# omnirevolve/omnirevolve-image-processor

Hardware: NVIDIA B200
Metric: megapixels/sec (resize+color+edge) (higher is better)
Workload: dtype u8

## Files before the change

### omnirevolve-image-processor_b200/csrc/capi.cu

```cuda
#include <stdlib.h>
#include "omni_internal.cuh"
#include "fast_kernels.cuh"
#include "fast_device.cuh"

#include <math.h>
#include <stdarg.h>
#include <stdio.h>
#include <string.h>

static thread_local char g_err[512] = "";

void omni_set_error(const char *fmt, ...)
{
    va_list ap;
    va_start(ap, fmt);
    vsnprintf(g_err, sizeof(g_err), fmt, ap);
    va_end(ap);
}

extern "C" const char *omni_last_error_string(void) { return g_err; }
extern "C" int omni_version(void) { return OMNI_ABI_VERSION; }

extern "C" int omni_device_count(void)
{
    int n = 0;
    if (cudaGetDeviceCount(&n) != cudaSuccess) { cudaGetLastError(); return 0; }
    return n;
}

extern "C" int omni_ctx_create(int device, omni_ctx **out)
{
    OMNI_REQUIRE(out != nullptr, "omni_ctx_create: out is NULL");
    int n = 0;
    cudaError_t e = cudaGetDeviceCount(&n);
    if (e != cudaSuccess || n == 0) {
        omni_set_error("no CUDA device available (%s); libomni_b200 has no CPU fallback",
                       e != cudaSuccess ? cudaGetErrorString(e) : "device count 0");
        cudaGetLastError();
        return OMNI_ERR_CUDA;
    }
    OMNI_REQUIRE(device >= 0 && device < n, "omni_ctx_create: device %d out of range [0,%d)", device, n);
    OMNI_CUDA(cudaSetDevice(device));
    omni_ctx *c = new omni_ctx();
    c->device = device;
    {
        const char *ev = getenv("OMNI_B200_EDGE_DENSE");
        c->edge_sparse = (ev && ev[0] == '1') ? 0 : 1;
        ev = getenv("OMNI_B200_ASSIGN_LABCELL");
        c->assign_rgbcell = (ev && ev[0] == '1') ? 0 : 1;
        ev = getenv("OMNI_B200_DENSE_PIPELINE");
        c->pipeline = (ev && ev[0] == '1') ? 0 : 1;
    }
    OMNI_CUDA(cudaMalloc(&c->d_flags, 64 * sizeof(int)));
    OMNI_CUDA(cudaMemset(c->d_flags, 0, 64 * sizeof(int)));
    OMNI_CUDA(cudaMalloc(&c->d_counts, 4 * OMNI_MAX_K * sizeof(unsigned long long)));
    OMNI_CUDA(cudaHostAlloc(&c->h_flags, 64 * sizeof(int), cudaHostAllocDefault));
    OMNI_CUDA(cudaHostAlloc(&c->h_counts, 4 * OMNI_MAX_K * sizeof(unsigned long long), cudaHostAllocDefault));
    OMNI_CUDA(cudaStreamCreateWithFlags(&c->stream, cudaStreamNonBlocking));
    OMNI_CUDA(cudaDeviceGetAttribute(&c->sm_count, cudaDevAttrMultiProcessorCount, device));
    *out = c;
    return OMNI_OK;
}

extern "C" int omni_ctx_destroy(omni_ctx *c)
{
    if (!c) return OMNI_OK;
    cudaSetDevice(c->device);
    for (int i = 0; i < OMNI_WS_SLOTS; i++) if (c->ws[i]) cudaFree(c->ws[i]);
    for (auto &kv : c->resize_tabs) if (kv.second.d_blob) cudaFree(kv.second.d_blob);
    if (c->d_flags) cudaFree(c->d_flags);
    if (c->d_rgb_boxes) cudaFree(c->d_rgb_boxes);
    if (c->d_rgb_boxes3) cudaFree(c->d_rgb_boxes3);
    if (c->d_counts) cudaFree(c->d_counts);
    if (c->h_flags) cudaFreeHost(c->h_flags);
    if (c->h_counts) cudaFreeHost(c->h_counts);
    if (c->stream) cudaStreamDestroy(c->stream);
    for (auto &r : c->prof) { cudaEventDestroy(r.a); cudaEventDestroy(r.b); }
    for (auto e : c->ev_pool) cudaEventDestroy(e);
    fast_ctx_release(c);
    if (c->pk_ready) {
        cudaStreamDestroy(c->pk_in); cudaStreamDestroy(c->pk_out);
        for (auto e : c->pk_ev) cudaEventDestroy(e);
    }
    if (c->pk_counts) cudaFreeHost(c->pk_counts);
    if (c->bd_ready) { for (auto e : c->bd_ev) cudaEventDestroy(e); cudaStreamDestroy(c->bd_tail); }
    if (c->band_helper) omni_ctx_destroy(c->band_helper);
    delete c;
    return OMNI_OK;
}

extern "C" int omni_set_fast_path(omni_ctx *ctx, int enable)
{
    OMNI_REQUIRE(ctx != nullptr, "omni_set_fast_path: ctx is NULL");
    ctx->fast = enable ? 1 : 0;
    if (enable) {
        ctx->edge_sparse = ctx->assign_rgbcell = (enable == 2) ? 0 : 1;
        ctx->pipeline = (enable == 1) ? 1 : 0;
    }
    return OMNI_OK;
}

extern "C" int omni_set_assume_binary_masks(omni_ctx *ctx, int enable)
{
    OMNI_REQUIRE(ctx != nullptr, "omni_set_assume_binary_masks: ctx is NULL");
    ctx->assume_binary = enable ? 1 : 0;
    return OMNI_OK;
}

extern "C" int omni_set_table_cache(omni_ctx *ctx, int enable)
{
    OMNI_REQUIRE(ctx != nullptr, "omni_set_table_cache: ctx is NULL");
    ctx->table_cache = enable ? 1 : 0;
    if (!enable) ctx->cells_valid = ctx->cells3_valid = 0;
    return OMNI_OK;
}

extern "C" int omni_set_host_bands(omni_ctx *ctx, int mode)
{
    OMNI_REQUIRE(ctx != nullptr, "ctx is NULL");
    OMNI_REQUIRE(mode >= 0 && mode <= 2, "omni_set_host_bands: mode must be 0, 1 or 2");
    ctx->host_bands = mode;
    return OMNI_OK;
}

extern "C" int omni_last_band_resends(omni_ctx *ctx) { return ctx ? ctx->last_band_resends : -1; }

extern "C" int omni_host_alloc(size_t bytes, void **out)
{
    OMNI_REQUIRE(out != nullptr, "omni_host_alloc: out is NULL");
    OMNI_CUDA(cudaHostAlloc(out, bytes ? bytes : 1, cudaHostAllocDefault));
    return OMNI_OK;
}

extern "C" int omni_host_free(void *p)
{
    if (p) OMNI_CUDA(cudaFreeHost(p));
    return OMNI_OK;
}

extern "C" int omni_last_hysteresis_passes(omni_ctx *ctx)
{
    if (!ctx) return 0;
    if (ctx->last_hyst_passes < 0) {
        cudaStream_t st = ctx->last_hyst_stream;
        if (cudaSetDevice(ctx->device) != cudaSuccess ||
            cudaMemcpyAsync(ctx->h_flags + 9, ctx->d_flags, sizeof(int), cudaMemcpyDeviceToHost, st) != cudaSuccess ||
            cudaStreamSynchronize(st) != cudaSuccess) {
            cudaGetLastError();
            return 0;
        }
        ctx->last_hyst_passes = ctx->h_flags[9];
    }
    return ctx->last_hyst_passes;
}

KScope::KScope(omni_ctx *ctx, const char *name, cudaStream_t s) : c(ctx), st(s)
// ... 903 lines not shown
```

### omnirevolve-image-processor_b200/csrc/fast_kernels.cu

```cuda
#include "fast_kernels.cuh"
#include "omni_tables.inc"
#include "fast_device.cuh"

#include <algorithm>
#include <type_traits>
#include <cooperative_groups.h>
#include <math.h>
#include <stdlib.h>
#include <string.h>
namespace cg = cooperative_groups;

#define FK_TRY(expr) do { int rc__ = (expr); if (rc__ != OMNI_OK) return rc__; } while (0)

__device__ u16 f_lab_tab[256 + 2048];
static bool f_tab_ready[64] = {false};

cudaError_t fast_tables()
{
    int dev = 0;
    cudaError_t e = cudaGetDevice(&dev);
    if (e != cudaSuccess) return e;
    if (dev < 64 && f_tab_ready[dev]) return cudaSuccess;
    e = cudaMemcpyToSymbol(f_lab_tab, OMNI_LAB_GAMMA, sizeof(OMNI_LAB_GAMMA), 0);
    if (e != cudaSuccess) return e;
// ... 798 lines not shown
                if (++run == R.maxt) emit();
            } else {
                if (run) emit();
                if (active && R.zero_fill) {
                    const int ty1 = min(y1, ty0 + ET_R);
                    for (int y = ty0; y < ty1; y++) {
                        const size_t o = (size_t)k * plane + (size_t)y * ws + c;
                        R.cbits[o] = 0u; R.sbits[o] = 0u;
                        if (R.edges) store_word_bytes(R.edges + (size_t)k * R.estride + (size_t)y * R.epitch, 32 * c, w, 0u, R.aligned16);
                    }
                }
            }
        }
        if (run) emit();
#pragma unroll
        for (int nt = 1; nt <= ET_MAXT; nt++) {
            int mine = 0;
            for (int i = 0; i < n_items; i++) mine += ((lens >> (3 * i)) & 7u) == (u32)nt;
            int x = mine;
#pragma unroll
            for (int d = 1; d < 32; d <<= 1) {
                int y = __shfl_up_sync(0xffffffffu, x, d);
                if (lane >= d) x += y;
            }
            const int total = __shfl_sync(0xffffffffu, x, 31);
            if (total == 0) continue;
            int base = 0;
            if (lane == 31) base = atomicAdd(R.run_counts + nt - 1, total);
            base = __shfl_sync(0xffffffffu, base, 31);
            int pos = base + x - mine;
            for (int i = 0; i < n_items; i++)
                if (((lens >> (3 * i)) & 7u) == (u32)nt) R.run_items[R.off.v[nt - 1] + pos++] = s_item[wid][i][lane];
        }
    }
}

static cudaError_t launch_morph(bool with02, int morph03, const u32 *in_bits, u32 *out_bits, const BitGeom &g, int K, u8 *masks,
                                size_t mstride, size_t mpitch, cudaStream_t st, int y_lo = 0, int y_hi = -1, const MorphRuns *runs = nullptr)
{
    if (y_hi < 0) y_hi = g.h;
    if (y_hi <= y_lo) return cudaSuccess;
    auto warps_at = [&](int tr) { return (long long)((g.ww + 127) / 128) * 4 * ((y_hi - y_lo + tr - 1) / tr) * K; };
    int tr = MORPH_TR;
    if (warps_at(MORPH_TR_BIG) >= MORPH_BIG_MIN_WARPS && (y_lo % MORPH_TR_BIG) == 0) tr = MORPH_TR_BIG;
    else if (warps_at(MORPH_TR_MID) >= MORPH_MID_MIN_WARPS && (y_lo % MORPH_TR_MID) == 0) tr = MORPH_TR_MID;
    dim3 b(128), grid((g.ww + 127) / 128, (y_hi - y_lo + tr - 1) / tr, K);
    int al = plane_align(masks, mstride, mpitch);
    MorphRuns R{};
    if (runs) R = *runs;
#define LM2(CODE, TAP, RUNS, TR) fk_morph<CODE, TAP, RUNS, TR><<<grid, b, 0, st>>>(in_bits, out_bits, g.ws, g.plane, g.h, g.w, masks, mstride, mpitch, al, y_lo, y_hi, R)
#define LM3(CODE, TAP, RUNS)                                                          \
    do {                                                                               \
        if (tr == MORPH_TR_BIG) LM2(CODE, TAP, RUNS, MORPH_TR_BIG);                    \
        else if (tr == MORPH_TR_MID) LM2(CODE, TAP, RUNS, MORPH_TR_MID);               \
        else LM2(CODE, TAP, RUNS, MORPH_TR);                                           \
    } while (0)
#define LM(CODE, TAP)                                                                  \
    do {                                                                               \
        if (runs) LM3(CODE, TAP, true); else LM3(CODE, TAP, false);                    \
    } while (0)
    if (with02) {
        switch (morph03) {
        case 0: LM(CODE_R_OC, 4); break;
        case 1: LM(CODE_F_O, 4); break;
        case 2: LM(CODE_F_C, 4); break;
        default: LM(CODE_F_OC, 4); break;
        }
    } else {
        switch (morph03) {
        case 1: LM(CODE_C_O, -1); break;
        case 2: LM(CODE_C_C, -1); break;
        case 3: LM(CODE_C_OC, -1); break;
        default: return cudaErrorInvalidValue;
        }
    }
#undef LM
#undef LM3
#undef LM2
    return cudaGetLastError();
}

#define HB_TR 32
#define HB_TW 32
#define HY_WORD_ROUNDS 4
#define HY_THREADS 1024

__device__ __forceinline__ void hy_patch_bytes(u8 *row, u32 promoted)
{
    if (row == nullptr) return;
    while (promoted) {
        int e = __ffs(promoted) - 1;
        promoted &= promoted - 1u;
        row[e] = 255;
    }
}

__device__ __forceinline__ int hy_worklist(u32 *__restrict__ ebits, const u32 *__restrict__ cbits, int ws, size_t plane, int h, int w, int n_weak,
                                   const u32 *__restrict__ worklist, u8 *__restrict__ edges, size_t estride, size_t epitch)
{
    const int wwl = (w + 31) >> 5;
    int rounds = 0;
    for (;;) {
        int changed = 0;
        for (int i = threadIdx.x; i < n_weak; i += HY_THREADS) {
            const u32 o = worklist[i];
            const int k = (int)(o / plane), rem = (int)(o - (size_t)k * plane);
            const int y = rem / ws, c = rem - y * ws;
            u32 *E = ebits + (size_t)k * plane + (size_t)y * ws;
            const u32 cv = __ldg(cbits + o);
            u32 m3[3], l3[3], r3[3];
#pragma unroll
            for (int dy = -1; dy <= 1; dy++) {
                const bool in = y + dy >= 0 && y + dy < h;
                const u32 *Er = E + (ptrdiff_t)dy * ws;
                m3[dy + 1] = in ? __ldcg(Er + c) : 0u;
                l3[dy + 1] = (in && c > 0) ? __ldcg(Er + c - 1) : 0u;
                r3[dy + 1] = (in && c + 1 < wwl) ? __ldcg(Er + c + 1) : 0u;
            }
            const u32 ev = m3[1];
            if ((cv & ~ev) == 0u) continue;
            u32 d = 0u;
#pragma unroll
            for (int q = 0; q < 3; q++) d |= m3[q] | (m3[q] << 1) | (m3[q] >> 1) | (l3[q] >> 31) | (r3[q] << 31);
            u32 nv = ev | (cv & d);
            for (;;) {
                u32 t = nv | (cv & ((nv << 1) | (nv >> 1)));
                if (t == nv) break;
                nv = t;
            }
            if (nv != ev) {
                E[c] = nv;
                changed = 1;
                hy_patch_bytes(edges ? edges + (size_t)k * estride + (size_t)y * epitch + 32 * c : nullptr, nv & ~ev);
            }
        }
        rounds++;
        __threadfence_block();
        if (!__syncthreads_or(changed)) break;
    }
    return rounds;
}

__global__ void __launch_bounds__(HY_THREADS) fk_hysteresis_wl(u32 *__restrict__ ebits, const u32 *__restrict__ cbits, int ws, size_t plane, int h,
                                                               int w, const int *flags, const u32 *__restrict__ worklist)
{
    const int n_weak = flags[4];
    if (n_weak > HY_WL_CAP) return;
    hy_worklist(ebits, cbits, ws, plane, h, w, n_weak, worklist, nullptr, 0, 0);
}

__global__ void __launch_bounds__(HY_THREADS) fk_hysteresis(u32 *__restrict__ ebits, const u32 *__restrict__ cbits, int ws, size_t plane, int h,
                                                     int w, int K, int *flags ,
                                                     const u32 *__restrict__ worklist,
                                                     u8 *__restrict__ edges, size_t estride, size_t epitch)
{
    cg::grid_group grid = cg::this_grid();
    const int n_weak = flags[4];
    if (n_weak <= HY_WL_CAP) {
        if (blockIdx.x != 0) return;
        const int rounds = hy_worklist(ebits, cbits, ws, plane, h, w, n_weak, worklist, edges, estride, epitch);
        if (threadIdx.x == 0) flags[0] = rounds;
        return;
    }
    __shared__ u32 s_e[(HB_TR + 2) * (HB_TW + 2)];
    __shared__ u32 s_c[HB_TR * HB_TW];
    const int ww = (w + 31) >> 5;
    const int tid = threadIdx.x;
    constexpr int SW = HB_TW + 2;
    int round = 0;
    for (;;) {
        volatile int *chg = flags + 1 + (round % 3);
        if (round < HY_WORD_ROUNDS) {
            const long long rows = (long long)K * h;
            const int lane = tid & 31;
            const long long warp0 = ((long long)blockIdx.x * blockDim.x + tid) >> 5, nwarps = ((long long)gridDim.x * blockDim.x) >> 5;
            for (long long R = warp0; R < rows; R += nwarps) {
                const int k = (int)(R / h), y = (int)(R - (long long)k * h);
                u32 *E = ebits + (size_t)k * plane + (size_t)y * ws;
                const u32 *C = cbits + (size_t)k * plane + (size_t)y * ws;
                for (int c = lane; c < ww; c += 32) {
                    const u32 cv = __ldg(C + c), ev = __ldcg(E + c);
                    if ((cv & ~ev) == 0u) continue;
                    u32 d = 0u;
#pragma unroll
                    for (int dy = -1; dy <= 1; dy++) {
                        if (y + dy < 0 || y + dy >= h) continue;
                        const u32 *Er = E + (ptrdiff_t)dy * ws;
                        u32 m = __ldcg(Er + c), l = c > 0 ? __ldcg(Er + c - 1) : 0u, r = c + 1 < ww ? __ldcg(Er + c + 1) : 0u;
                        d |= m | (m << 1) | (m >> 1) | (l >> 31) | (r << 31);
                    }
                    u32 nv = ev | (cv & d);
                    for (;;) {
                        u32 t = nv | (cv & ((nv << 1) | (nv >> 1)));
                        if (t == nv) break;
                        nv = t;
                    }
                    if (nv != ev) {
                        E[c] = nv;
                        *chg = 1;
                        hy_patch_bytes(edges ? edges + (size_t)k * estride + (size_t)y * epitch + 32 * c : nullptr, nv & ~ev);
                    }
                }
            }
        } else {
            const int tx_n = (ww + HB_TW - 1) / HB_TW, ty_n = (h + HB_TR - 1) / HB_TR;
            const int tiles = tx_n * ty_n * K;
            for (int t = blockIdx.x; t < tiles; t += gridDim.x) {
                const int k = t / (tx_n * ty_n), r = t - k * (tx_n * ty_n);
                const int ty = r / tx_n, tx = r - ty * tx_n;
                const int y0 = ty * HB_TR, c0 = tx * HB_TW;
                u32 *E = ebits + (size_t)k * plane;
                const u32 *C = cbits + (size_t)k * plane;
                int pending = 0;
                for (int i = tid; i < HB_TR * HB_TW; i += HY_THREADS) {
                    int ly = i / HB_TW, lc = i - ly * HB_TW;
                    int gy = y0 + ly, gc = c0 + lc;
                    u32 cv = 0, ev = 0;
                    if (gy < h && gc < ww) { cv = __ldg(C + (size_t)gy * ws + gc); ev = __ldcg(E + (size_t)gy * ws + gc); }
                    s_c[i] = cv;
                    s_e[(ly + 1) * SW + lc + 1] = ev;
                    pending |= (cv & ~ev) != 0;
                }
                if (!__syncthreads_or(pending)) continue;
                for (int i = tid; i < 2 * SW + 2 * HB_TR; i += HY_THREADS) {
                    int ly, lc;
                    if (i < SW) { ly = 0; lc = i; }
                    else if (i < 2 * SW) { ly = HB_TR + 1; lc = i - SW; }
                    else { int j = i - 2 * SW; ly = 1 + (j >> 1); lc = (j & 1) ? HB_TW + 1 : 0; }
                    int gy = y0 - 1 + ly, gc = c0 - 1 + lc;
                    s_e[ly * SW + lc] = (gy >= 0 && gy < h && gc >= 0 && gc < ww) ? __ldcg(E + (size_t)gy * ws + gc) : 0u;
                }
                __syncthreads();
                int any = 0;
                for (;;) {
                    int changed = 0;
                    for (int i = tid; i < HB_TR * HB_TW; i += HY_THREADS) {
                        int ly = i / HB_TW, lc = i - ly * HB_TW;
                        u32 cv = s_c[i];
                        int o = (ly + 1) * SW + lc + 1;
                        u32 ev = s_e[o];
                        if (cv & ~ev) {
                            u32 d = 0;
#pragma unroll
                            for (int dy = -1; dy <= 1; dy++) {
                                u32 l = s_e[o + dy * SW - 1], m = s_e[o + dy * SW], rr = s_e[o + dy * SW + 1];
                                d |= m | (m << 1) | (m >> 1) | (l >> 31) | (rr << 31);
                            }
                            u32 nv = ev | (cv & d);
                            if (nv != ev) { s_e[o] = nv; changed = 1; }
                        }
                    }
                    if (!__syncthreads_or(changed)) break;
                    any = 1;
                }
                if (any) {
                    for (int i = tid; i < HB_TR * HB_TW; i += HY_THREADS) {
                        int ly = i / HB_TW, lc = i - ly * HB_TW;
                        int gy = y0 + ly, gc = c0 + lc;
                        if (gy < h && gc < ww) {
                            u32 nv = s_e[(ly + 1) * SW + lc + 1], old = __ldcg(E + (size_t)gy * ws + gc);
                            if (nv & ~old) {
                                E[(size_t)gy * ws + gc] = nv | old;
                                hy_patch_bytes(edges ? edges + (size_t)k * estride + (size_t)gy * epitch + 32 * gc : nullptr, nv & ~old);
                            }
                        }
                    }
                    if (tid == 0) *chg = 1;
                }
                __syncthreads();
            }
        }
        __threadfence();
        grid.sync();
        const int c = *chg;
        if (blockIdx.x == 0 && tid == 0) { flags[0] = round + 1; flags[1 + ((round + 2) % 3)] = 0; }
        round++;
        if (!c) break;
    }
}

#define HP_MAX_BANDS 8
static int pipe_init(omni_ctx *ctx);
int persist_blocks(omni_ctx *ctx, int per_sm) { return (ctx->sm_count > 0 ? ctx->sm_count : 148) * per_sm; }

template <typename Kern>
static int resident_grid(omni_ctx *ctx, Kern kern, int block, int *cache)
{
    if (*cache == 0) {
        int per_sm = 0;
        if (cudaOccupancyMaxActiveBlocksPerMultiprocessor(&per_sm, kern, block, 0) != cudaSuccess || per_sm < 1) {
            cudaGetLastError();
            per_sm = 1;
        }
        *cache = per_sm;
    }
    return persist_blocks(ctx, *cache);
}

static int bit_planes(omni_ctx *ctx, const BitGeom &g, int K, int n, u32 **out )
{
    size_t one = g.plane * (size_t)K * sizeof(u32);
    one = (one + 255) & ~(size_t)255;
    FK_TRY(omni_ws_reserve(ctx, 4, one * n));
    for (int i = 0; i < n; i++) out[i] = (u32 *)((u8 *)ctx->ws[4] + one * i);
    return OMNI_OK;
}

void dense_ws_bytes(int h, int w, int K, int nf, int ksize, size_t out[OMNI_WS_SLOTS])
{
    const BitGeom g = make_geom(h, w);
    const int KT = nf * K;
    size_t one = (g.plane * (size_t)KT * sizeof(u32) + 255) & ~(size_t)255;
    unsigned off[ET_MAXT];
    out[4] = std::max(out[4], one * 4);
    out[5] = std::max(out[5], WS5_BYTES);
    out[6] = std::max(out[6], edges3_run_words(h, w, KT, off) * sizeof(u32));
    out[2] = std::max(out[2], (((size_t)w + 15) & ~(size_t)15) * h);
    if (ksize != 3) out[0] = std::max(out[0], (((size_t)w + 15) & ~(size_t)15) * h * KT);
}

bool lut_below_k(const AssignParams &P)
{
    for (int k = 0; k < P.K; k++)
        if (P.lut[k] >= P.K) return false;
    return true;
}

static int assign_cells(omni_ctx *ctx, const AssignParams &P, u32 **cells, u8 **rcells, cudaStream_t st)
{
    FK_TRY(omni_ws_reserve(ctx, 5, WS5_BYTES));
    const int variant = (ctx->assign_rgbcell && P.K <= RC_MAX_K && lut_below_k(P)) ? 2 : 1;
    *cells = (u32 *)ctx->ws[5];
    *rcells = (u8 *)((u32 *)ctx->ws[5] + RGBCELL_OFFSET);
    if (ctx->table_cache && ctx->cells_valid == variant && ctx->cells_stream == (void *)st && ctx->cells_K == P.K &&
        memcmp(ctx->cells_c, P.c, sizeof(float) * 3 * P.K) == 0 && memcmp(ctx->cells_lut, P.lut, P.K) == 0)
        return OMNI_OK;
    memcpy(ctx->cells_c, P.c, sizeof(float) * 3 * P.K);
    memcpy(ctx->cells_lut, P.lut, P.K);
    ctx->cells_K = P.K; ctx->cells_stream = (void *)st; ctx->cells_valid = variant;
    {
        KScope ks(ctx, "build_cells", st);
        fk_build_cells<<<CELL_COUNT / 256, 256, 0, st>>>(P, *cells);
        OMNI_CUDA(cudaGetLastError());
    }
    if (variant == 2) {
        FK_TRY(fast_rgb_boxes(ctx, st));
        KScope ks(ctx, "build_rgbcells", st);
        fk_build_rgbcells<<<RC_COUNT / 8 / 256, 256, 0, st>>>(P, ctx->d_rgb_boxes, (u32 *)*rcells, *rcells + RC_NIB_BYTES);
        OMNI_CUDA(cudaGetLastError());
    }
    return OMNI_OK;
}

static bool assign_takes_zero_job(omni_ctx *ctx, const AssignParams &P, int nf, int h, int w)
{
    const unsigned long long plane = (unsigned long long)(((((w + 31) >> 5) + 3) & ~3)) * h;
    return ctx->assign_rgbcell && P.K <= RC_MAX_K && lut_below_k(P) && (long long)nf * h * ((w + 255) >> 8) < (1ll << 30) &&
           (unsigned long long)nf * P.K * plane < (1ull << 30);
}

// ... 60 lines not shown

bool fast_masks_supported(int open_iters, int close_iters)
{
    return (open_iters == 1 && close_iters == 1) || (open_iters <= 0 && close_iters <= 0);
}

int fast_layer_masks(omni_ctx *ctx, const u8 *d_labels, int h, int w, size_t lpitch, int K, int open_iters, int close_iters,
                     u8 *d_masks, size_t plane_stride, size_t mpitch, cudaStream_t st)
{
    BitGeom g = make_geom(h, w);
    u32 *bp[1];
    FK_TRY(bit_planes(ctx, g, K, 1, bp));
    {
        KScope ks(ctx, "labels_to_bits", st);
        fk_labels_to_bits<<<persist_blocks(ctx, 8), 256, 0, st>>>(d_labels, h, w, lpitch, K, bp[0], g.ws, g.plane);
        OMNI_CUDA(cudaGetLastError());
    }
    int al = plane_align(d_masks, plane_stride, mpitch);
    if (open_iters == 1 && close_iters == 1) {
        OMNI_LAUNCH(ctx, st, "morph_bits", launch_morph(true, 0, bp[0], nullptr, g, K, d_masks, plane_stride, mpitch, st));
    } else {
        KScope ks(ctx, "expand_bits", st);
        fk_expand_bits<<<dim3(persist_blocks(ctx, 4), K), 256, 0, st>>>(bp[0], g.ws, g.plane, h, w, d_masks, plane_stride, mpitch, al);
        OMNI_CUDA(cudaGetLastError());
    }
    return OMNI_OK;
}

int morph03_kind(const omni_edge_params *p)
{
    int oi = p->open_iters > 0 ? p->open_iters : 0, ci = p->close_iters > 0 ? p->close_iters : 0;
    if (p->morph_k == 1) return 0;
    if (p->morph_k != 3 || oi > 1 || ci > 1) return -1;
    return oi | (ci << 1);
}

static bool morph03_bits_ok(const omni_edge_params *p) { return morph03_kind(p) >= 0 || (p->morph_k >= 2 && p->morph_k <= OMNI_MAX_MORPH_K); }

bool fast_edges_supported(const omni_edge_params *prm)
{
    return morph03_bits_ok(prm) && (prm->ksize == 3 || prm->ksize == 5 || prm->ksize == 7);
}

bool fast_fused_supported(const omni_edge_params *prm) { return morph03_kind(prm) >= 0 && prm->ksize == 3; }

bool fast_morph03_supported(const omni_edge_params *prm) { return morph03_bits_ok(prm); }

int fast_morph03_bytes(omni_ctx *ctx, const u8 *d_masks, int K, int h, int w, size_t m_plane, size_t mpitch,
                       const omni_edge_params *prm, u8 *d_out, size_t o_plane, size_t opitch, cudaStream_t st)
{
    BitGeom g = make_geom(h, w);
    u32 *bpp[2];
    FK_TRY(bit_planes(ctx, g, K, 2, bpp));
    OMNI_CUDA(cudaMemsetAsync(ctx->d_flags + 8, 0, sizeof(int), st));
    {
        KScope ks(ctx, "bytes_to_bits", st);
        fk_bytes_to_bits<true><<<dim3(persist_blocks(ctx, 2), K), 256, 0, st>>>(d_masks, m_plane, mpitch, h, w, bpp[0], g.ws, g.plane,
                                                                               ctx->d_flags + 8);
        OMNI_CUDA(cudaGetLastError());
    }
    if (!ctx->assume_binary) {
        OMNI_CUDA(cudaMemcpyAsync(ctx->h_flags + 8, ctx->d_flags + 8, sizeof(int), cudaMemcpyDeviceToHost, st));
        OMNI_CUDA(cudaStreamSynchronize(st));
        if (ctx->h_flags[8]) return OMNI_ERR_UNSUPPORTED;
    }
    const int kind = morph03_kind(prm);
    const u32 *m2 = bpp[0];
    if (kind > 0) {
        OMNI_LAUNCH(ctx, st, "morph_bits", launch_morph(false, kind, bpp[0], bpp[1], g, K, nullptr, 0, 0, st));
        m2 = bpp[1];
    } else if (kind < 0) {
        FK_TRY(ellipse_morph_bits(ctx, prm, g, K, bpp[0], bpp[1], &m2, st));
    }
    int al = plane_align(d_out, o_plane, opitch);
    KScope ks(ctx, "expand_bits", st);
    fk_expand_bits<<<dim3(persist_blocks(ctx, 4), K), 256, 0, st>>>(m2, g.ws, g.plane, h, w, d_out, o_plane, opitch, al);
    OMNI_CUDA(cudaGetLastError());
    return OMNI_OK;
}

int run_hysteresis(omni_ctx *ctx, u32 *ebits, const u32 *cbits, const BitGeom &g, int K, u8 *d_edges,
                          size_t e_plane, size_t epitch, cudaStream_t st, int *flags_in, const u32 *worklist_in)
{
    if (ctx->hyst_blocks == 0) {
        int per_sm = 0;
        OMNI_CUDA(cudaOccupancyMaxActiveBlocksPerMultiprocessor(&per_sm, fk_hysteresis, HY_THREADS, 0));
        if (per_sm < 1) { omni_set_error("hysteresis kernel cannot be made resident"); return OMNI_ERR_CUDA; }
        ctx->hyst_blocks = per_sm * (ctx->sm_count > 0 ? ctx->sm_count : 1);
    }
    int ws = g.ws, h = g.h, w = g.w;
    size_t plane = g.plane;
    int *flags = flags_in ? flags_in : ctx->d_flags;
    const u32 *worklist = worklist_in ? worklist_in : (const u32 *)ctx->ws[5] + HYST_WL_OFFSET;
    void *args[] = {&ebits, &cbits, &ws, &plane, &h, &w, &K, &flags, &worklist, &d_edges, &e_plane, &epitch};
    OMNI_LAUNCH(ctx, st, "hysteresis_bits", cudaLaunchCooperativeKernel((const void *)fk_hysteresis, dim3(ctx->hyst_blocks), dim3(HY_THREADS),
                                                                        args, 0, st));
    if (!flags_in) {
        ctx->last_hyst_passes = -1;
        ctx->last_hyst_stream = st;
    }
    return OMNI_OK;
}

int run_hysteresis_wl(omni_ctx *ctx, u32 *ebits, const u32 *cbits, const BitGeom &g, int K, cudaStream_t st, const int *flags, const u32 *worklist)
{
    (void)K;
    KScope ks(ctx, "hysteresis_wl", st);
    fk_hysteresis_wl<<<1, HY_THREADS, 0, st>>>(ebits, cbits, g.ws, g.plane, g.h, g.w, flags, worklist);
    OMNI_CUDA(cudaGetLastError());
    return OMNI_OK;
}

int edge_pass_begin(omni_ctx *ctx, const BitGeom &g, int K, u32 *sbits, u32 *cbits, u8 *d_edges, size_t e_plane, size_t epitch,
                           cudaStream_t st, MorphRuns *R, bool *sparse, bool side_fill, ZeroJob *zjob)
{
    FK_TRY(omni_ws_reserve(ctx, 5, WS5_BYTES));
    OMNI_CUDA(cudaMemsetAsync(ctx->d_flags, 0, 24 * sizeof(int), st));
    ctx->edge_join = nullptr;
    *sparse = ctx->edge_sparse && edges3_sparse_ok(g.h, g.w, K);
    if (!*sparse) return OMNI_OK;
    if (ctx->e3s_per_sm == 0) ctx->e3s_per_sm = edges3_sparse_blocks_per_sm();
    FK_TRY(omni_ws_reserve(ctx, 6, edges3_run_words(g.h, g.w, K, R->off.v) * sizeof(u32)));
    R->sbits = sbits; R->cbits = cbits; R->edges = d_edges; R->estride = e_plane; R->epitch = epitch;
    R->aligned16 = plane_align(d_edges, e_plane, epitch);
    R->run_counts = ctx->d_flags + 16; R->run_items = (u32 *)ctx->ws[6];
    R->maxt = edges3_pick_maxt(g.h, g.w, K, 2 * persist_blocks(ctx, ctx->e3s_per_sm));
    R->zero_fill = side_fill ? 0 : 1;
    if (side_fill && zjob && epitch == (size_t)g.w && e_plane == epitch * (size_t)g.h && (uintptr_t)d_edges % 16 == 0 &&
        (e_plane * (size_t)K) % 16 == 0 && cbits == sbits + ((g.plane * (size_t)K * sizeof(u32) + 255) & ~(size_t)255) / sizeof(u32)) {
        zjob->p[0] = (uint4 *)d_edges; zjob->n16[0] = e_plane * (size_t)K / 16;
        zjob->p[1] = (uint4 *)sbits;   zjob->n16[1] = (size_t)((u8 *)cbits - (u8 *)sbits + g.plane * (size_t)K * sizeof(u32)) / 16;
        return OMNI_OK;
    }
    if (side_fill) {
        FK_TRY(pipe_init(ctx));
        cudaEvent_t fork = ctx->pipe_ev[2 * HP_MAX_BANDS + 4], join = ctx->pipe_ev[2 * HP_MAX_BANDS + 5];
        cudaStream_t ss = ctx->s_in;
        OMNI_CUDA(cudaEventRecord(fork, st));
        OMNI_CUDA(cudaStreamWaitEvent(ss, fork, 0));
        if (epitch == (size_t)g.w && e_plane == epitch * (size_t)g.h) OMNI_CUDA(cudaMemsetAsync(d_edges, 0, e_plane * (size_t)K, ss));
        else
            for (int k = 0; k < K; k++) OMNI_CUDA(cudaMemset2DAsync(d_edges + (size_t)k * e_plane, epitch, 0, (size_t)g.w, g.h, ss));
        const size_t pbytes = g.plane * (size_t)K * sizeof(u32);
        OMNI_CUDA(cudaMemsetAsync(sbits, 0, pbytes, ss));
        OMNI_CUDA(cudaMemsetAsync(cbits, 0, pbytes, ss));
        OMNI_CUDA(cudaEventRecord(join, ss));
        ctx->edge_join = join;
    }
    return OMNI_OK;
}

static int edges_from_bits(omni_ctx *ctx, const u32 *m2, u32 *sbits, u32 *cbits, const BitGeom &g, int K, int low, int high,
                           u8 *d_edges, size_t e_plane, size_t epitch, cudaStream_t st, bool sparse, bool runs_done,
                           const u8 *blur = nullptr , size_t bstride = 0, size_t bpitch = 0)
{
    int al = plane_align(d_edges, e_plane, epitch);
    if (ctx->edge_join) {
        OMNI_CUDA(cudaStreamWaitEvent(st, ctx->edge_join, 0));
        ctx->edge_join = nullptr;
    }
    if (sparse) {
        if (!runs_done)
            OMNI_LAUNCH(ctx, st, "edge_runs", launch_edge_runs(m2, g.ws, g.plane, g.h, g.w, K, sbits, cbits, d_edges, e_plane, epitch, al,
                                                               ctx->d_flags + 16, (u32 *)ctx->ws[6], 2 * persist_blocks(ctx, ctx->e3s_per_sm), st));
        OMNI_LAUNCH(ctx, st, "edges3_bits", launch_edges3_sparse(m2, g.ws, g.plane, g.h, g.w, K, low, high, persist_blocks(ctx, ctx->e3s_per_sm),
                                                                 sbits, cbits, d_edges, e_plane, epitch, al, ctx->d_flags + 4,
                                                                 (u32 *)ctx->ws[5] + HYST_WL_OFFSET, HY_WL_CAP, ctx->d_flags + 16,
                                                                 ctx->d_flags + 20, (const u32 *)ctx->ws[6], st, blur, bstride, bpitch));
    } else {
        OMNI_LAUNCH(ctx, st, "edges3_bits", launch_edges3_simd(m2, g.ws, g.plane, g.h, g.w, K, low, high, ctx->sm_count, sbits, cbits,
                                                               d_edges, e_plane, epitch, al, ctx->d_flags + 4,
                                                               (u32 *)ctx->ws[5] + HYST_WL_OFFSET, HY_WL_CAP, st, blur, bstride, bpitch));
    }
    return run_hysteresis(ctx, sbits, cbits, g, K, d_edges, e_plane, epitch, st);
}

int fast_edges(omni_ctx *ctx, const u8 *d_masks, int K, int h, int w, size_t m_plane, size_t mpitch,
               const omni_edge_params *prm, const BlurParams &bp, int low, int high,
               u8 *d_edges, size_t e_plane, size_t epitch, cudaStream_t st)
// ... 468 lines not shown
```

### omnirevolve-image-processor_b200/csrc/omni_internal.cuh

```cuda
#pragma once
#include <cuda_runtime.h>
#include <stdint.h>
#include <stddef.h>
#include <map>
#include <string>
#include <tuple>
#include <vector>

#include "../../include/omni_b200.h"

typedef uint8_t u8;
typedef uint16_t u16;
typedef uint32_t u32;
typedef uint64_t u64;

void omni_set_error(const char *fmt, ...);
#define OMNI_CUDA(call)                                                                         \
    do {                                                                                        \
        cudaError_t e__ = (call);                                                               \
        if (e__ != cudaSuccess) {                                                               \
            omni_set_error("%s:%d %s -> %s", __FILE__, __LINE__, #call, cudaGetErrorString(e__)); \
            return OMNI_ERR_CUDA;                                                               \
        }                                                                                       \
    } while (0)
#define OMNI_REQUIRE(cond, ...)                                                                 \
    do {                                                                                        \
        if (!(cond)) { omni_set_error(__VA_ARGS__); return OMNI_ERR_ARG; }                      \
    } while (0)

struct AssignParams {
    float c[OMNI_MAX_K * 3];
    u8 pal[OMNI_MAX_K * 3];
    u8 lut[OMNI_MAX_K];
    int K;
};
struct BlurParams {
    u16 w[OMNI_MAX_BLUR_K];
    int k;
};
struct MorphSE {
    int8_t x0[OMNI_MAX_MORPH_K];
    int8_t x1[OMNI_MAX_MORPH_K];
    int k;
};
struct ResizeTabDev {
    const int *xofs; const int *xsi; const float *xal;
    const int *yofs; const int *ysi; const float *yal;
};

struct ResizeTab {
    void *d_blob = nullptr;
    ResizeTabDev dev{};
};

#define OMNI_WS_SLOTS 11
struct omni_ctx {
    int device = 0;
    int fast = 1;
    void *ws[OMNI_WS_SLOTS] = {};
    size_t ws_bytes[OMNI_WS_SLOTS] = {};
    int *d_flags = nullptr;
    unsigned long long *d_counts = nullptr;
    int *h_flags = nullptr;
    unsigned long long *h_counts = nullptr;
    cudaStream_t stream = nullptr;
    std::map<std::tuple<int, int, int, int>, ResizeTab> resize_tabs;
    int last_hyst_passes = 0;
    cudaStream_t last_hyst_stream = nullptr;
    long long launches = 0;
    int prof_on = 0;
    struct ProfRec { const char *name; cudaEvent_t a, b; };
    std::vector<ProfRec> prof;
    std::vector<cudaEvent_t> ev_pool;
    int sm_count = 0;
    int hyst_blocks = 0;
    int thin_blocks = 0;
    int e3s_per_sm = 0;
    int assign_rgbcell = 1;
    int edge_sparse = 1;
    int assume_binary = 0;
    int pipe_ready = 0;
    cudaStream_t s_in = nullptr, s_out = nullptr;
    cudaEvent_t pipe_ev[24] = {};
    cudaEvent_t edge_join = nullptr;
    int occ_assign_lab = 0, occ_assign_pal = 0, occ_assign_rgb = 0, occ_assign_i16 = 0;
    int cells_valid = 0, cells_K = 0;
    void *cells_stream = nullptr;
    float cells_c[OMNI_MAX_K * 3];
    u8 cells_lut[OMNI_MAX_K] = {};
    int cells3_valid = 0, cells3_K = 0;
    void *cells3_stream = nullptr;
    float cells3_c[OMNI_MAX_K * 3];
    u8 cells3_lut[OMNI_MAX_K] = {};
    u8 *d_rgb_boxes3 = nullptr;
    int table_cache = 1;
    int tables_hold = 0;
    int occ_assign_sl = 0;
    int pk_ready = 0;
    cudaStream_t pk_in = nullptr, pk_out = nullptr;
    cudaEvent_t pk_ev[7] = {};
    cudaEvent_t bd_ev[3 * 16 + 2] = {};
    int bd_ready = 0;
    cudaStream_t bd_tail = nullptr;
    omni_ctx *band_helper = nullptr;
    int band_overlap = 1;
    int host_bands = 2;
    int last_band_resends = 0;
    unsigned long long *pk_counts = nullptr;
    size_t pk_counts_cap = 0;
    int pipeline = 1;
    u8 *d_rgb_boxes = nullptr;
    int trace_valid = 0, trace_K = 0;
    long long trace_points = 0, trace_paths = 0;
    std::vector<long long> trace_info;
    std::vector<int32_t> trace_comp;
};

struct KScope {
    omni_ctx *c; cudaStream_t st; cudaEvent_t b = nullptr;
    KScope(omni_ctx *ctx, const char *name, cudaStream_t s);
    ~KScope();
};
#define OMNI_LAUNCH(ctx, st, name, expr) do { KScope ks__(ctx, name, st); OMNI_CUDA(expr); } while (0)

int omni_ws_reserve(omni_ctx *ctx, int slot, size_t bytes);
int trace_run(omni_ctx *ctx, const u8 *d_skel, int K, int h, int w, size_t plane_stride, size_t pitch, int64_t *h_info,
              cudaStream_t st);
int trace_results(omni_ctx *ctx, int32_t *points, int32_t *path_len, int32_t *comp);
const ResizeTab *omni_get_resize_tab(omni_ctx *ctx, int sh, int sw, int dh, int dw, cudaStream_t st);
void omni_build_se(int shape_ellipse, int k, MorphSE *se);
int omni_gauss_weights(int k, BlurParams *bp);

cudaError_t g_resize_area(const u8 *src, int sh, int sw, size_t spitch, u8 *dst, int dh, int dw, size_t dpitch,
                          const ResizeTabDev *tab, cudaStream_t st);
cudaError_t g_assign(const u8 *px, int h, int w, size_t pitch, const AssignParams &P, int mode_lab,
                     u8 *labels, size_t lpitch, cudaStream_t st);
cudaError_t g_onehot(const u8 *labels, int h, int w, size_t lpitch, int K, u8 *planes, size_t plane_stride,
                     size_t pitch, cudaStream_t st);
cudaError_t g_morph(const u8 *src, size_t s_plane, size_t spitch, u8 *dst, size_t d_plane, size_t dpitch,
                    int K, int h, int w, const MorphSE &se, int is_dilate, cudaStream_t st);
cudaError_t g_blur(const u8 *src, size_t s_plane, size_t spitch, u8 *dst, size_t d_plane, size_t dpitch,
                   int K, int h, int w, const BlurParams &bp, cudaStream_t st);
cudaError_t g_canny_nms(const u8 *src, size_t s_plane, size_t spitch, u8 *state, size_t d_plane, size_t dpitch,
                        int K, int h, int w, int low, int high, cudaStream_t st);
cudaError_t g_hyst_pass(u8 *state, size_t plane, size_t pitch, int K, int h, int w, int *d_changed, cudaStream_t st);
cudaError_t g_hyst_final(u8 *state, size_t plane, size_t pitch, int K, int h, int w, cudaStream_t st);
cudaError_t g_count_nonzero(const u8 *planes, size_t plane, size_t pitch, int K, int h, int w,
                            unsigned long long *d_counts, cudaStream_t st);
cudaError_t g_count_labels(const u8 *labels, size_t pitch, int h, int w, int K, unsigned long long *d_counts,
                           cudaStream_t st);
cudaError_t g_composite(const u8 *edges, size_t plane, size_t pitch, int K, int h, int w, const u8 *colors_bgr,
                        u8 *canvas, size_t cpitch, cudaStream_t st);
cudaError_t g_skeleton_degree(const u8 *skel, size_t s_plane, size_t spitch, int K, int h, int w, u8 *deg, size_t d_plane, size_t dpitch,
                              u8 *nodes, size_t n_plane, size_t npitch, cudaStream_t st);
cudaError_t g_pack_bytes(const u8 *src, size_t s_plane, size_t spitch, int K, int h, int w, u8 *dst, size_t d_plane, size_t dpitch,
                         int msb_first, unsigned long long *counts, cudaStream_t st);
cudaError_t g_copy2d_planes(const u8 *src, size_t s_plane, size_t spitch, u8 *dst, size_t d_plane, size_t dpitch,
                            int K, int h, int w, cudaStream_t st);
// ... 79 lines not shown
```

Baseline: 45770.

## Replace cooperative grid-sync hysteresis with persistent tile work-queue propagation

The hysteresis kernel no longer uses a cooperative launch that alternates global word-rounds and tile rounds separated by grid.sync. It now runs as a persistent kernel: blocks first claim every tile once, then pull dirty tiles from a device-side ring queue. Neighbour tiles are re-enqueued only when promoted bits reach their border, and the last block to finish resets the counters. This removes full-grid barriers and repeated sweeps over clean tiles, at the cost of atomic contention, spin-waiting on the queue, and the risk of subtle races in the hand-written lock-free queue.

```diff
diff --git a/omnirevolve-image-processor_b200/csrc/capi.cu b/omnirevolve-image-processor_b200/csrc/capi.cu
--- a/omnirevolve-image-processor_b200/csrc/capi.cu
+++ b/omnirevolve-image-processor_b200/csrc/capi.cu
@@ -72,6 +72,7 @@
     if (c->d_rgb_boxes) cudaFree(c->d_rgb_boxes);
     if (c->d_rgb_boxes3) cudaFree(c->d_rgb_boxes3);
     if (c->d_counts) cudaFree(c->d_counts);
+    if (c->d_hyq) cudaFree(c->d_hyq);
     if (c->h_flags) cudaFreeHost(c->h_flags);
     if (c->h_counts) cudaFreeHost(c->h_counts);
     if (c->stream) cudaStreamDestroy(c->stream);
diff --git a/omnirevolve-image-processor_b200/csrc/fast_kernels.cu b/omnirevolve-image-processor_b200/csrc/fast_kernels.cu
--- a/omnirevolve-image-processor_b200/csrc/fast_kernels.cu
+++ b/omnirevolve-image-processor_b200/csrc/fast_kernels.cu
@@ -904,8 +904,15 @@
 
 #define HB_TR 32
 #define HB_TW 32
-#define HY_WORD_ROUNDS 4
 #define HY_THREADS 1024
+#define HYQ_CTRS 8
+
+struct HyQueue {
+    unsigned long long *ctr;
+    unsigned long long *ring;
+    unsigned *queued;
+    unsigned n;
+};
 
 __device__ __forceinline__ void hy_patch_bytes(u8 *row, u32 promoted)
 {
@@ -971,12 +978,123 @@
     hy_worklist(ebits, cbits, ws, plane, h, w, n_weak, worklist, nullptr, 0, 0);
 }
 
+__device__ void hy_push(const HyQueue &Q, unsigned t, unsigned gen)
+{
+    if (atomicExch(Q.queued + t, 1u) != 0u) return;
+    atomicAdd(Q.ctr + 3, 1ull);
+    atomicMax(Q.ctr + 4, (unsigned long long)gen);
+    __threadfence();
+    const unsigned long long slot = atomicAdd(Q.ctr + 1, 1ull) % Q.n;
+    while (atomicCAS(Q.ring + slot, 0ull, ((unsigned long long)gen << 32) | (t + 1u)) != 0ull) __nanosleep(32);
+}
+
+__device__ unsigned long long hy_pop(const HyQueue &Q)
+{
+    volatile unsigned long long *c = Q.ctr;
+    for (;;) {
+        const unsigned long long tail = c[2];
+        if (tail < c[1]) {
+            if (atomicCAS(Q.ctr + 2, tail, tail + 1) != tail) continue;
+            unsigned long long v;
+            while ((v = atomicExch(Q.ring + tail % Q.n, 0ull)) == 0ull) __nanosleep(32);
+            atomicExch(Q.queued + (unsigned)(v & 0xffffffffu) - 1u, 0u);
+            __threadfence();
+            return v;
+        }
+        if (c[3] == 0ull) return 0ull;
+        __nanosleep(128);
+    }
+}
+
+__device__ void hy_tile(u32 *__restrict__ ebits, const u32 *__restrict__ cbits, int ws, size_t plane, int h, int ww, int tx_n, int ty_n,
+                        unsigned t, unsigned gen, const HyQueue &Q, u8 *__restrict__ edges, size_t estride, size_t epitch,
+                        u32 *s_e, u32 *s_c, unsigned *s_dirs)
+{
+    constexpr int SW = HB_TW + 2;
+    const int tid = threadIdx.x;
+    const int k = t / (tx_n * ty_n), r = t - k * (tx_n * ty_n);
+    const int ty = r / tx_n, tx = r - ty * tx_n;
+    const int y0 = ty * HB_TR, c0 = tx * HB_TW;
+    u32 *E = ebits + (size_t)k * plane;
+    const u32 *C = cbits + (size_t)k * plane;
+    int pending = 0;
+    for (int i = tid; i < HB_TR * HB_TW; i += HY_THREADS) {
+        int ly = i / HB_TW, lc = i - ly * HB_TW;
+        int gy = y0 + ly, gc = c0 + lc;
+        u32 cv = 0, ev = 0;
+        if (gy < h && gc < ww) { cv = __ldg(C + (size_t)gy * ws + gc); ev = __ldcg(E + (size_t)gy * ws + gc); }
+        s_c[i] = cv;
+        s_e[(ly + 1) * SW + lc + 1] = ev;
+        pending |= (cv & ~ev) != 0;
+    }
+    if (tid == 0) *s_dirs = 0u;
+    if (!__syncthreads_or(pending)) return;
+    for (int i = tid; i < 2 * SW + 2 * HB_TR; i += HY_THREADS) {
+        int ly, lc;
+        if (i < SW) { ly = 0; lc = i; }
+        else if (i < 2 * SW) { ly = HB_TR + 1; lc = i - SW; }
+        else { int j = i - 2 * SW; ly = 1 + (j >> 1); lc = (j & 1) ? HB_TW + 1 : 0; }
+        int gy = y0 - 1 + ly, gc = c0 - 1 + lc;
+        s_e[ly * SW + lc] = (gy >= 0 && gy < h && gc >= 0 && gc < ww) ? __ldcg(E + (size_t)gy * ws + gc) : 0u;
+    }
+    __syncthreads();
+    int any = 0;
+    for (;;) {
+        int changed = 0;
+        for (int i = tid; i < HB_TR * HB_TW; i += HY_THREADS) {
+            int ly = i / HB_TW, lc = i - ly * HB_TW;
+            u32 cv = s_c[i];
+            int o = (ly + 1) * SW + lc + 1;
+            u32 ev = s_e[o];
+            if (cv & ~ev) {
+                u32 d = 0;
+#pragma unroll
+                for (int dy = -1; dy <= 1; dy++) {
+                    u32 l = s_e[o + dy * SW - 1], m = s_e[o + dy * SW], rr = s_e[o + dy * SW + 1];
+                    d |= m | (m << 1) | (m >> 1) | (l >> 31) | (rr << 31);
+                }
+                u32 nv = ev | (cv & d);
+                if (nv != ev) { s_e[o] = nv; changed = 1; }
+            }
+        }
+        if (!__syncthreads_or(changed)) break;
+        any = 1;
+    }
+    if (!any) return;
+    unsigned dirs = 0u;
+    for (int i = tid; i < HB_TR * HB_TW; i += HY_THREADS) {
+        int ly = i / HB_TW, lc = i - ly * HB_TW;
+        int gy = y0 + ly, gc = c0 + lc;
+        if (gy >= h || gc >= ww) continue;
+        const u32 nv = s_e[(ly + 1) * SW + lc + 1];
+        u32 *e = E + (size_t)gy * ws + gc;
+        if ((nv & ~__ldcg(e)) == 0u) continue;
+        const u32 p = nv & ~atomicOr(e, nv);
+        if (p == 0u) continue;
+        hy_patch_bytes(edges ? edges + (size_t)k * estride + (size_t)gy * epitch + 32 * gc : nullptr, p);
+        const unsigned rows = 2u | (ly == 0 ? 1u : 0u) | (ly == HB_TR - 1 ? 4u : 0u);
+        const unsigned cols = 2u | ((lc == 0 && (p & 1u)) ? 1u : 0u) | ((lc == HB_TW - 1 && (p >> 31)) ? 4u : 0u);
+#pragma unroll
+        for (int dy = 0; dy < 3; dy++)
+            if ((rows >> dy) & 1u) dirs |= (cols & 7u) << (3 * dy);
+    }
+    dirs &= ~(1u << 4);
+    if (dirs) atomicOr(s_dirs, dirs);
+    __threadfence();
+    __syncthreads();
+    if (tid == 0) {
+        for (unsigned d = *s_dirs; d; d &= d - 1u) {
+            const int b = __ffs(d) - 1, ny = ty + b / 3 - 1, nx = tx + b % 3 - 1;
+            if (ny >= 0 && ny < ty_n && nx >= 0 && nx < tx_n) hy_push(Q, (unsigned)(k * tx_n * ty_n + ny * tx_n + nx), gen + 1u);
+        }
+    }
+}
+
 __global__ void __launch_bounds__(HY_THREADS) fk_hysteresis(u32 *__restrict__ ebits, const u32 *__restrict__ cbits, int ws, size_t plane, int h,
                                                      int w, int K, int *flags ,
                                                      const u32 *__restrict__ worklist,
-                                                     u8 *__restrict__ edges, size_t estride, size_t epitch)
-{
-    cg::grid_group grid = cg::this_grid();
+                                                     u8 *__restrict__ edges, size_t estride, size_t epitch, HyQueue Q)
+{
     const int n_weak = flags[4];
     if (n_weak <= HY_WL_CAP) {
         if (blockIdx.x != 0) return;
@@ -986,118 +1104,38 @@
     }
     __shared__ u32 s_e[(HB_TR + 2) * (HB_TW + 2)];
     __shared__ u32 s_c[HB_TR * HB_TW];
+    __shared__ unsigned s_dirs;
+    __shared__ unsigned long long s_item;
     const int ww = (w + 31) >> 5;
-    const int tid = threadIdx.x;
-    constexpr int SW = HB_TW + 2;
-    int round = 0;
+    const int tx_n = (ww + HB_TW - 1) / HB_TW, ty_n = (h + HB_TR - 1) / HB_TR;
+    const unsigned tiles = (unsigned)(tx_n * ty_n * K);
     for (;;) {
-        volatile int *chg = flags + 1 + (round % 3);
-        if (round < HY_WORD_ROUNDS) {
-            const long long rows = (long long)K * h;
-            const int lane = tid & 31;
-            const long long warp0 = ((long long)blockIdx.x * blockDim.x + tid) >> 5, nwarps = ((long long)gridDim.x * blockDim.x) >> 5;
-            for (long long R = warp0; R < rows; R += nwarps) {
-                const int k = (int)(R / h), y = (int)(R - (long long)k * h);
-                u32 *E = ebits + (size_t)k * plane + (size_t)y * ws;
-                const u32 *C = cbits + (size_t)k * plane + (size_t)y * ws;
-                for (int c = lane; c < ww; c += 32) {
-                    const u32 cv = __ldg(C + c), ev = __ldcg(E + c);
-                    if ((cv & ~ev) == 0u) continue;
-                    u32 d = 0u;
-#pragma unroll
-                    for (int dy = -1; dy <= 1; dy++) {
-                        if (y + dy < 0 || y + dy >= h) continue;
-                        const u32 *Er = E + (ptrdiff_t)dy * ws;
-                        u32 m = __ldcg(Er + c), l = c > 0 ? __ldcg(Er + c - 1) : 0u, r = c + 1 < ww ? __ldcg(Er + c + 1) : 0u;
-                        d |= m | (m << 1) | (m >> 1) | (l >> 31) | (r << 31);
-                    }
-                    u32 nv = ev | (cv & d);
-                    for (;;) {
-                        u32 t = nv | (cv & ((nv << 1) | (nv >> 1)));
-                        if (t == nv) break;
-                        nv = t;
-                    }
-                    if (nv != ev) {
-                        E[c] = nv;
-                        *chg = 1;
-                        hy_patch_bytes(edges ? edges + (size_t)k * estride + (size_t)y * epitch + 32 * c : nullptr, nv & ~ev);
-                    }
-                }
-            }
-        } else {
-            const int tx_n = (ww + HB_TW - 1) / HB_TW, ty_n = (h + HB_TR - 1) / HB_TR;
-            const int tiles = tx_n * ty_n * K;
-            for (int t = blockIdx.x; t < tiles; t += gridDim.x) {
-                const int k = t / (tx_n * ty_n), r = t - k * (tx_n * ty_n);
-                const int ty = r / tx_n, tx = r - ty * tx_n;
-                const int y0 = ty * HB_TR, c0 = tx * HB_TW;
-                u32 *E = ebits + (size_t)k * plane;
-                const u32 *C = cbits + (size_t)k * plane;
-                int pending = 0;
-                for (int i = tid; i < HB_TR * HB_TW; i += HY_THREADS) {
-                    int ly = i / HB_TW, lc = i - ly * HB_TW;
-                    int gy = y0 + ly, gc = c0 + lc;
-                    u32 cv = 0, ev = 0;
-                    if (gy < h && gc < ww) { cv = __ldg(C + (size_t)gy * ws + gc); ev = __ldcg(E + (size_t)gy * ws + gc); }
-                    s_c[i] = cv;
-                    s_e[(ly + 1) * SW + lc + 1] = ev;
-                    pending |= (cv & ~ev) != 0;
-                }
-                if (!__syncthreads_or(pending)) continue;
-                for (int i = tid; i < 2 * SW + 2 * HB_TR; i += HY_THREADS) {
-                    int ly, lc;
-                    if (i < SW) { ly = 0; lc = i; }
-                    else if (i < 2 * SW) { ly = HB_TR + 1; lc = i - SW; }
-                    else { int j = i - 2 * SW; ly = 1 + (j >> 1); lc = (j & 1) ? HB_TW + 1 : 0; }
-                    int gy = y0 - 1 + ly, gc = c0 - 1 + lc;
-                    s_e[ly * SW + lc] = (gy >= 0 && gy < h && gc >= 0 && gc < ww) ? __ldcg(E + (size_t)gy * ws + gc) : 0u;
-                }
-                __syncthreads();
-                int any = 0;
-                for (;;) {
-                    int changed = 0;
-                    for (int i = tid; i < HB_TR * HB_TW; i += HY_THREADS) {
-                        int ly = i / HB_TW, lc = i - ly * HB_TW;
-                        u32 cv = s_c[i];
-                        int o = (ly + 1) * SW + lc + 1;
-                        u32 ev = s_e[o];
-                        if (cv & ~ev) {
-                            u32 d = 0;
-#pragma unroll
-                            for (int dy = -1; dy <= 1; dy++) {
-                                u32 l = s_e[o + dy * SW - 1], m = s_e[o + dy * SW], rr = s_e[o + dy * SW + 1];
-                                d |= m | (m << 1) | (m >> 1) | (l >> 31) | (rr << 31);
-                            }
-                            u32 nv = ev | (cv & d);
-                            if (nv != ev) { s_e[o] = nv; changed = 1; }
-                        }
-                    }
-                    if (!__syncthreads_or(changed)) break;
-                    any = 1;
-                }
-                if (any) {
-                    for (int i = tid; i < HB_TR * HB_TW; i += HY_THREADS) {
-                        int ly = i / HB_TW, lc = i - ly * HB_TW;
-                        int gy = y0 + ly, gc = c0 + lc;
-                        if (gy < h && gc < ww) {
-                            u32 nv = s_e[(ly + 1) * SW + lc + 1], old = __ldcg(E + (size_t)gy * ws + gc);
-                            if (nv & ~old) {
-                                E[(size_t)gy * ws + gc] = nv | old;
-                                hy_patch_bytes(edges ? edges + (size_t)k * estride + (size_t)gy * epitch + 32 * gc : nullptr, nv & ~old);
-                            }
-                        }
-                    }
-                    if (tid == 0) *chg = 1;
-                }
-                __syncthreads();
-            }
-        }
+        if (threadIdx.x == 0) s_item = atomicAdd(Q.ctr + 0, 1ull);
+        __syncthreads();
+        const unsigned long long t = s_item;
+        __syncthreads();
+        if (t >= tiles) break;
+        hy_tile(ebits, cbits, ws, plane, h, ww, tx_n, ty_n, (unsigned)t, 0u, Q, edges, estride, epitch, s_e, s_c, &s_dirs);
+        __syncthreads();
+    }
+    for (;;) {
+        if (threadIdx.x == 0) s_item = hy_pop(Q);
+        __syncthreads();
+        const unsigned long long v = s_item;
+        __syncthreads();
+        if (v == 0ull) break;
+        hy_tile(ebits, cbits, ws, plane, h, ww, tx_n, ty_n, (unsigned)(v & 0xffffffffu) - 1u, (unsigned)(v >> 32), Q, edges, estride, epitch,
+                s_e, s_c, &s_dirs);
+        __syncthreads();
+        if (threadIdx.x == 0) atomicAdd(Q.ctr + 3, ~0ull);
+    }
+    if (threadIdx.x != 0) return;
+    __threadfence();
+    if (atomicAdd(Q.ctr + 5, 1ull) == gridDim.x - 1) {
         __threadfence();
-        grid.sync();
-        const int c = *chg;
-        if (blockIdx.x == 0 && tid == 0) { flags[0] = round + 1; flags[1 + ((round + 2) % 3)] = 0; }
-        round++;
-        if (!c) break;
+        volatile unsigned long long *c = Q.ctr;
+        flags[0] = 1 + (int)c[4];
+        for (int i = 0; i < HYQ_CTRS; i++) c[i] = 0ull;
     }
 }
 
@@ -1324,19 +1362,24 @@
 int run_hysteresis(omni_ctx *ctx, u32 *ebits, const u32 *cbits, const BitGeom &g, int K, u8 *d_edges,
                           size_t e_plane, size_t epitch, cudaStream_t st, int *flags_in, const u32 *worklist_in)
 {
-    if (ctx->hyst_blocks == 0) {
-        int per_sm = 0;
-        OMNI_CUDA(cudaOccupancyMaxActiveBlocksPerMultiprocessor(&per_sm, fk_hysteresis, HY_THREADS, 0));
-        if (per_sm < 1) { omni_set_error("hysteresis kernel cannot be made resident"); return OMNI_ERR_CUDA; }
-        ctx->hyst_blocks = per_sm * (ctx->sm_count > 0 ? ctx->sm_count : 1);
-    }
-    int ws = g.ws, h = g.h, w = g.w;
-    size_t plane = g.plane;
+    const unsigned tiles = (unsigned)K * (unsigned)((g.h + HB_TR - 1) / HB_TR) * (unsigned)((g.ww + HB_TW - 1) / HB_TW);
+    if (ctx->hyq_tiles < tiles) {
+        if (ctx->d_hyq) { OMNI_CUDA(cudaFree(ctx->d_hyq)); ctx->d_hyq = nullptr; ctx->hyq_tiles = 0; }
+        const size_t bytes = (HYQ_CTRS + (size_t)tiles) * sizeof(unsigned long long) + (size_t)tiles * sizeof(unsigned);
+        OMNI_CUDA(cudaMalloc(&ctx->d_hyq, bytes));
+        OMNI_CUDA(cudaMemsetAsync(ctx->d_hyq, 0, bytes, st));
+        ctx->hyq_tiles = tiles;
+    }
+    HyQueue Q;
+    Q.ctr = (unsigned long long *)ctx->d_hyq;
+    Q.ring = Q.ctr + HYQ_CTRS;
+    Q.queued = (unsigned *)(Q.ring + ctx->hyq_tiles);
+    Q.n = tiles;
     int *flags = flags_in ? flags_in : ctx->d_flags;
     const u32 *worklist = worklist_in ? worklist_in : (const u32 *)ctx->ws[5] + HYST_WL_OFFSET;
-    void *args[] = {&ebits, &cbits, &ws, &plane, &h, &w, &K, &flags, &worklist, &d_edges, &e_plane, &epitch};
-    OMNI_LAUNCH(ctx, st, "hysteresis_bits", cudaLaunchCooperativeKernel((const void *)fk_hysteresis, dim3(ctx->hyst_blocks), dim3(HY_THREADS),
-                                                                        args, 0, st));
+    OMNI_LAUNCH(ctx, st, "hysteresis_bits", (fk_hysteresis<<<persist_blocks(ctx, 1), HY_THREADS, 0, st>>>(ebits, cbits, g.ws, g.plane, g.h, g.w, K, flags,
+                                                                                          worklist, d_edges, e_plane, epitch, Q),
+                                             cudaGetLastError()));
     if (!flags_in) {
         ctx->last_hyst_passes = -1;
         ctx->last_hyst_stream = st;
diff --git a/omnirevolve-image-processor_b200/csrc/omni_internal.cuh b/omnirevolve-image-processor_b200/csrc/omni_internal.cuh
--- a/omnirevolve-image-processor_b200/csrc/omni_internal.cuh
+++ b/omnirevolve-image-processor_b200/csrc/omni_internal.cuh
@@ -73,7 +73,8 @@
     std::vector<ProfRec> prof;
     std::vector<cudaEvent_t> ev_pool;
     int sm_count = 0;
-    int hyst_blocks = 0;
+    void *d_hyq = nullptr;
+    unsigned hyq_tiles = 0;
     int thin_blocks = 0;
     int e3s_per_sm = 0;
     int assign_rgbcell = 1;
```

After: 45590, median of 6. No clear change (-0.4%).
